# at-wat/mcl_3dl

Hardware: AMD Instinct MI355X
Metric: particle·point evals/sec; filter-update Hz @ 4096 particles × 16k-pt scan (higher is better)
Workload: dtype f32

## Files before the change

include/mcl3dl_hip.h:

```cpp
#ifndef MCL3DL_HIP_H
#define MCL3DL_HIP_H

#include <stddef.h>
#include <stdint.h>

#ifdef __cplusplus
extern "C" {
#endif

#define MCL3DL_HIP_ABI_VERSION 3

typedef struct mcl3dl_hip_ctx mcl3dl_hip_ctx;

enum
{
  MCL3DL_BEAM_SHORT = 0,
  MCL3DL_BEAM_HIT = 1,
  MCL3DL_BEAM_LONG = 2,
  MCL3DL_BEAM_TOTAL_REFLECTION = 3
};

enum
{
  MCL3DL_KERNEL_LIKELIHOOD = 0,
// ... 206 lines not shown
int mcl3dl_hip_group_measure_imu(mcl3dl_hip_group* g, const float* acc3, float acc_var, float* out_weight ,
                                 float* out_lik , float* entropy, int* restored);
int mcl3dl_hip_group_set_odom_error_sigma(mcl3dl_hip_group* g, float sigma);
int mcl3dl_hip_global_localization_rotations(int div_yaw, const float* imu_quat4 ,
                                             float* out_quat4 );
int mcl3dl_hip_global_localization_points(mcl3dl_hip_ctx* ctx, double grid, float* out_xyz ,
                                          size_t capacity, size_t* n_points, size_t* n_centroids);
int mcl3dl_hip_global_localization_seed_device(mcl3dl_hip_ctx* ctx, int div_yaw, const float* imu_quat4, size_t first,
                                               size_t count, float* d_state13, float* d_pose7, float* d_weight);
int mcl3dl_hip_group_global_localization(mcl3dl_hip_group* g, double grid, int div_yaw, const float* imu_quat4,
                                         size_t max_particles , size_t* n_points, size_t* n_particles);
int mcl3dl_hip_sampler_normal_direction(const float* mean7 , const float* cov36 ,
                                        double perform_weighting_ratio, double max_weight_ratio, double max_weight,
                                        float* out_fpc_local3, double* out_max_weight, double* out_eigen_value_ratio );
int mcl3dl_hip_scan_normal_weights(mcl3dl_hip_ctx* ctx, int which, double normal_search_range, const float* fpc_local3,
                                   double max_weight, double* out_cumulative , float* out_normal_xyz ,
                                   size_t capacity, size_t* n, size_t* n_without_normal );
int mcl3dl_hip_group_collective_stats(const mcl3dl_hip_group* g, uint64_t* rccl_all_reduces, uint64_t* host_combines);

int mcl3dl_hip_set_kernel_timing(mcl3dl_hip_ctx* ctx, int enable);
int mcl3dl_hip_get_kernel_time(mcl3dl_hip_ctx* ctx, int kernel_id, double* total_ms, uint64_t* launches);
int mcl3dl_hip_reset_kernel_time(mcl3dl_hip_ctx* ctx);
int mcl3dl_hip_workload_stats(mcl3dl_hip_ctx* ctx, const float* d_pose, size_t n_p, double* stats6);
int mcl3dl_hip_memory_footprint(mcl3dl_hip_ctx* ctx, uint64_t* bytes8);
int mcl3dl_hip_set_option(mcl3dl_hip_ctx* ctx, const char* name, double value);
int mcl3dl_hip_get_option(mcl3dl_hip_ctx* ctx, const char* name, double* value);
int mcl3dl_hip_index_stats(mcl3dl_hip_ctx* ctx, double* stats8);

#ifdef __cplusplus
}
#endif
#endif
```

mcl_3dl_amd/capi.py:

```python
import ctypes as C
import os

import numpy as np

_HERE = os.path.dirname(os.path.abspath(__file__))
LIB_PATH = os.environ.get("MCL3DL_HIP_LIB") or os.path.join(_HERE, "libmcl3dl_hip.so")

KERNEL_LIKELIHOOD, KERNEL_BEAM, KERNEL_PF, KERNEL_UPDATE, KERNEL_STAGE = 0, 1, 2, 3, 4
BEAM_STATUS = {0: "SHORT", 1: "HIT", 2: "LONG", 3: "TOTAL_REFLECTION"}

_f, _d, _sz, _u32, _u64, _i, _p = C.c_float, C.c_double, C.c_size_t, C.c_uint32, C.c_uint64, C.c_int, C.c_void_p

SIGNATURES = {
    "mcl3dl_hip_abi_version": (_i, []),
    "mcl3dl_hip_create": (_i, [C.POINTER(_p), _i]),
    "mcl3dl_hip_destroy": (None, [_p]),
    "mcl3dl_hip_last_error": (C.c_char_p, [_p]),
    "mcl3dl_hip_set_stream": (_i, [_p, _p]),
    "mcl3dl_hip_get_stream": (_p, [_p]),
    "mcl3dl_hip_synchronize": (_i, [_p]),
    "mcl3dl_hip_set_map": (_i, [_p, _p, _p, _sz, _u64, _p]),
    "mcl3dl_hip_set_likelihood_params": (_i, [_p, _f, _f, _f]),
    "mcl3dl_hip_set_beam_params": (_i, [_p, _f, _f, _f, _f, _f, _f, _f, _u32, _f, _u32, _i]),
    "mcl3dl_hip_set_beam_raycast": (_i, [_p, _i]),
# ... 17 lines not shown
    "mcl3dl_hip_expectation": (_i, [_p, _p, _p, _p, _sz, _p, _p, _p, _p]),
    "mcl3dl_hip_covariance": (_i, [_p, _p, _p, _sz, _p, _sz, _p, _p]),
    "mcl3dl_hip_expectation_device": (_i, [_p, _p, _p, _p, _sz, _p, _p, _p, _p]),
    "mcl3dl_hip_covariance_device": (_i, [_p, _p, _p, _sz, _p, _sz, _p, _p]),
    "mcl3dl_hip_resample_begin": (_i, [_p, _p, _sz, _sz, C.POINTER(_f)]),
    "mcl3dl_hip_resample_plan": (_i, [_p, _i, _f, _p, _p, C.POINTER(_sz)]),
    "mcl3dl_hip_resample_apply": (_i, [_p, _p, _p, _sz, _p]),
    "mcl3dl_hip_resample_apply_device": (_i, [_p, _p, _p, _sz, _p]),
    "mcl3dl_hip_moments_partial_device": (_i, [_p, _p, _p, _p, _sz, _p]),
    "mcl3dl_hip_moments_finish": (_i, [_p, _i, _p, _p, C.POINTER(_f), C.POINTER(C.c_int64), C.POINTER(C.c_int64)]),
    "mcl3dl_hip_covariance_partial_device": (_i, [_p, _p, _p, _sz, _p, _sz, _p, _p]),
    "mcl3dl_hip_covariance_finish": (_i, [_p, _p]),
    "mcl3dl_hip_update_device": (_i, [_p, _p, _sz, _p, _p, _p, _p, _p, _p]),
    "mcl3dl_hip_resample_begin_device": (_i, [_p, _p, _sz, _sz, C.POINTER(_f)]),
    "mcl3dl_hip_resample_apply_slice_device": (_i, [_p, _p, _p, _sz, _sz, _sz, _p]),
    "mcl3dl_hip_upload_scan": (_i, [_p, _p, _sz, _p, _p, _sz, _p, _sz]),
    "mcl3dl_hip_measure_device": (_i, [_p, _p, _sz, _p, _p, _p]),
    "mcl3dl_hip_pf_partial_device": (_i, [_p, _p, _p, _p, _p, _p, _sz, _i, _i, _p]),
    "mcl3dl_hip_pf_apply_device": (_i, [_p, _p, _sz, _i, _p, _p]),
    "mcl3dl_hip_set_kernel_timing": (_i, [_p, _i]),
    "mcl3dl_hip_get_kernel_time": (_i, [_p, _i, C.POINTER(_d), C.POINTER(_u64)]),
    "mcl3dl_hip_reset_kernel_time": (_i, [_p]),
    "mcl3dl_hip_workload_stats": (_i, [_p, _p, _sz, _p]),
    "mcl3dl_hip_memory_footprint": (_i, [_p, _p]),
    "mcl3dl_hip_set_option": (_i, [_p, C.c_char_p, _d]),
    "mcl3dl_hip_scan_begin": (_i, [_p, _p, _p, _sz, _p, _p, _p, C.POINTER(_sz), C.POINTER(_sz), C.POINTER(_sz)]),
    "mcl3dl_hip_scan_begin_pointcloud2": (_i, [_p, _p, _sz, _u32, _i, _i, _i, _i, _u32, _p, _p, _p, C.POINTER(_sz),
                                              C.POINTER(_sz), C.POINTER(_sz)]),
    "mcl3dl_hip_scan_finish": (_i, [_p, _p, _sz, _p, _sz, _p, _sz]),
    "mcl3dl_hip_scan_download": (_i, [_p, _i, _p, _p, _sz, C.POINTER(_sz)]),
    "mcl3dl_hip_set_map_pointcloud2": (_i, [_p, _p, _sz, _u32, _i, _i, _i, _i, _p, _u64, _p, C.POINTER(_sz)]),
    "mcl3dl_hip_set_map_downsampled": (_i, [_p, _p, _p, _sz, _p, _u64, _p, C.POINTER(_sz)]),
    "mcl3dl_hip_map_update": (_i, [_p, _p, _p, _sz, _p, _u64, C.POINTER(_sz), _p]),
    "mcl3dl_hip_map_update_pointcloud2": (_i, [_p, _p, _sz, _u32, _i, _i, _i, _i, _p, _u64, C.POINTER(_sz), _p]),
    "mcl3dl_hip_map_download": (_i, [_p, _p, _p, _sz, C.POINTER(_sz)]),
    "mcl3dl_hip_match_split": (_i, [_p, _p, _p, _sz, _f, _d, _p, _sz, C.POINTER(_sz), _p, _sz, C.POINTER(_sz)]),
    "mcl3dl_hip_group_create": (_i, [C.POINTER(_p), C.POINTER(_i), _i]),
    "mcl3dl_hip_group_destroy": (None, [_p]),
    "mcl3dl_hip_group_last_error": (C.c_char_p, [_p]),
    "mcl3dl_hip_group_size": (_i, [_p]),
    "mcl3dl_hip_group_context": (_p, [_p, _i]),
    "mcl3dl_hip_group_shard": (_i, [_sz, _i, _i, C.POINTER(_sz), C.POINTER(_sz)]),
    "mcl3dl_hip_group_set_map": (_i, [_p, _p, _p, _sz, _u64, _p]),
    "mcl3dl_hip_group_set_likelihood_params": (_i, [_p, _f, _f, _f]),
    "mcl3dl_hip_group_set_beam_params": (_i, [_p, _f, _f, _f, _f, _f, _f, _f, _u32, _f, _u32, _i]),
    "mcl3dl_hip_group_set_beam_raycast": (_i, [_p, _i]),
# ... 838 lines not shown
                                                          _ptr(d_extra), _ptr(d_ratio), n_p, int(rank), int(world),
                                                          _ptr(d_packed)))

    def pf_apply_device(self, d_weight, n_p, d_packed, d_stats4, world=1):
        self._check(self.lib.mcl3dl_hip_pf_apply_device(self.h, _ptr(d_weight), n_p, int(world), _ptr(d_packed),
                                                        _ptr(d_stats4)))

    def set_kernel_timing(self, enable):
        self._check(self.lib.mcl3dl_hip_set_kernel_timing(self.h, int(bool(enable))))

    def reset_kernel_time(self):
        self._check(self.lib.mcl3dl_hip_reset_kernel_time(self.h))

    def kernel_time(self, kernel_id):
        ms, n = C.c_double(0), C.c_uint64(0)
        self._check(self.lib.mcl3dl_hip_get_kernel_time(self.h, kernel_id, C.byref(ms), C.byref(n)))
        return float(ms.value), int(n.value)

    def workload_stats(self, d_pose, n_p):
        st = np.zeros(6, np.float64)
        self._check(self.lib.mcl3dl_hip_workload_stats(self.h, _ptr(d_pose), n_p, _ptr(st)))
        return dict(sum_k=st[0], evals=st[1], dda_steps=st[2], dda_occupied=st[3], dda_tested=st[4], rays=st[5])

    def memory_footprint(self):
        b = np.zeros(8, np.uint64)
        self._check(self.lib.mcl3dl_hip_memory_footprint(self.h, _ptr(b)))
        return dict(lik_points=int(b[0]), lik_cells=int(b[1]), dda_bits=int(b[2]), dda_voxels=int(b[3]),
                    dda_points=int(b[4]), cand_table=int(b[5]), cand_start=int(b[6]), cand_points=int(b[7]))

    def set_option(self, name, value):
        self._check(self.lib.mcl3dl_hip_set_option(self.h, name.encode(), float(value)))

    def get_option(self, name):
        v = C.c_double(0)
        self._check(self.lib.mcl3dl_hip_get_option(self.h, name.encode(), C.byref(v)))
        return float(v.value)

    def index_stats(self):
        s = np.zeros(8, np.float64)
        self._check(self.lib.mcl3dl_hip_index_stats(self.h, _ptr(s)))
        return dict(bricks=int(s[0]), preliminary=int(s[1]), candidates=int(s[2]), build_ms=float(s[3]),
                    voxels_with_candidates=int(s[4]), voxels_with_overflow=int(s[5]), overflow_records=int(s[6]),
                    voxel_ratio=float(s[7]), voxels_over8=int(self.get_option("cand_voxels_over8")),
                    record_parts=int(self.get_option("cand_record_parts_in_use")),
                    packed_words=int(self.get_option("cand_packed_active")),
                    deferred_overflow=int(self.get_option("lik_defer_active")))
# ... 1 lines not shown
```

mcl_3dl_amd/csrc/grid_kernels.h:

```cpp
#pragma once
#include <hip/hip_runtime.h>
#include <stdint.h>

#include "map_structs.h"
#pragma clang fp contract(off)

namespace mcl3dl
{
__global__ void grid_rescale_kernel(const float4* __restrict__ map, long long n, float wx, float wy, float wz, int has_weight,
                                    float4* __restrict__ out)
{
  const long long i = static_cast<long long>(blockIdx.x) * blockDim.x + threadIdx.x;
  if (i >= n)
    return;
  const float4 p = map[i];
  out[i] = make_float4(has_weight ? p.x * wx : p.x, has_weight ? p.y * wy : p.y, has_weight ? p.z * wz : p.z,
                       __uint_as_float(static_cast<uint32_t>(i)));
}

struct CellGeom
{
  float ox, oy, oz, inv;
  int nx, ny, nz;
};
// ... 181 lines not shown
  unsigned long long bit;
  dda_brick_bit(g, v, brick, bit);
  atomicAnd(&bricks[brick], ~bit);
}

__global__ void dda_overlay_set_kernel(const float4* __restrict__ upd, const uint32_t* __restrict__ skey,
                                       const uint32_t* __restrict__ sval, int n, DdaGeom g, uint32_t* __restrict__ ov_key,
                                       float4* __restrict__ ov_pts, uint32_t* __restrict__ ov_idx,
                                       unsigned long long* __restrict__ bricks)
{
  const int k = static_cast<int>(blockIdx.x * blockDim.x + threadIdx.x);
  if (k >= n)
    return;
  const uint32_t v = skey[k], i = sval[k];
  ov_key[k] = v;
  ov_pts[k] = upd[i];
  ov_idx[k] = i;
  size_t brick;
  unsigned long long bit;
  dda_brick_bit(g, v, brick, bit);
  atomicOr(&bricks[brick], bit);
}

}
```

mcl_3dl_amd/csrc/host_context.h:

```cpp
#pragma once

namespace
{
struct DevBuf
{
  void* p = nullptr;
  size_t cap = 0;
  bool view = false;
  DevBuf() = default;
  DevBuf(const DevBuf&) = delete;
  DevBuf& operator=(const DevBuf&) = delete;
  ~DevBuf()
  {
    if (p && !view)
      (void)hipFree(p);
  }
  template <typename T>
  T* as() const
  {
    return static_cast<T*>(p);
  }
};

struct OrderedScan
// ... 126 lines not shown
    for (const PinnedBlock& b : pinned)
      if (c >= b.p && c + bytes <= b.p + b.bytes)
        return true;
    return false;
  }
  double cand_voxel_ratio = 0.0;
  double cand_phase = 0.5;
  int cand_aniso = 2;
  bool cand_aniso_active = false;
  double cand_aniso_max = 8.0;
  double index_budget_opt = -1.0;
  double index_budget_bytes = 0.0;
  double cand_need_bytes = 0.0;
  double cand_edge_ratio[3] = { 0.5, 0.5, 0.5 };
  int cand_record_parts = 0;
  uint32_t cand_parts = 4;
  int n_cus = 256;
  int cand_packed = 1;
  int cand_bound = 1;
  int lik_defer = 1;
  double lik_defer_min_frac = 0.03;
  double cand_over8 = 0;
  DevBuf cand_table, cand_start, cand_pts, cand_rec, cand_ovf;
  DevBuf cand_all_pts;
  CompileParams cand_cp{};
  long long cand_n_table = 0;
  uint32_t cand_n_bricks = 0, cand_n_ovf = 0, cand_ovf_leaked = 0;
  uint64_t cand_ovf_compactions = 0;
  size_t cand_n_points = 0;
  RecGrid rg{};
  double cand_stats[8] = { 0, 0, 0, 0, 0, 0, 0, 0 };
  DevBuf dda_bits, dda_start, dda_pts, dda_index;
  DevBuf dda_ov_key, dda_ov_pts, dda_ov_idx;
  int dda_overlay = 1;
  bool dda_overlay_ok = false;
  uint64_t dda_overlay_updates = 0;
  DdaGeom dda_geom{};
  DevBuf map_dev;
  bool map_dev_valid = false;
  size_t map_dev_n = 0;
  int grid_build_host = 0;
  double grid_build_ms[2] = { 0, 0 };
  double grid_build_wall_ms[2] = { 0, 0 };
  DdaGrid dg{};
  uint64_t footprint[8] = { 0, 0, 0, 0, 0, 0, 0, 0 };

// ... 568 lines not shown
```

mcl_3dl_amd/csrc/host_map_compilers.h:

```cpp
#pragma once

namespace
{
int build_lik_grid(mcl3dl_hip_ctx* ctx);
int build_dda_grid(mcl3dl_hip_ctx* ctx);
int ensure_map_dev(mcl3dl_hip_ctx* ctx);
int cloud_minmax(mcl3dl_hip_ctx* ctx, const float4* pts, long long n, float* host6, unsigned long long* host_cnt);

void kd_ray_radii(const mcl3dl_hip_ctx* ctx, float* grid_min, float* r1, float* r2)
{
  const float mn = std::min({ ctx->map_grid[0], ctx->map_grid[1], ctx->map_grid[2] });
  const float mx = std::max({ ctx->map_grid[0], ctx->map_grid[1], ctx->map_grid[2] });
  *grid_min = mn;
  *r1 = static_cast<float>(std::sqrt(2.0) * mx / 2.0);
  *r2 = static_cast<float>(mn * 2 + std::sqrt(2.0) * mx / 2.0);
}

bool lik_cell_is_beams(const mcl3dl_hip_ctx* ctx)
{
  return !ctx->lik_params_set && ctx->beam_raycast == 1;
}

float lik_cell_edge(const mcl3dl_hip_ctx* ctx)
{
// ... 363 lines not shown
{
  sp.resize(count);
  for (size_t k = 0; k < count; ++k)
  {
    const size_t i = first + k;
    float v[3];
    for (int a = 0; a < 3; ++a)
    {
      v[a] = ctx->has_weight ? ctx->map_xyz[3 * i + a] * ctx->weight[a] : ctx->map_xyz[3 * i + a];
      if (!std::isfinite(v[a]))
        return ctx->fail(-3, "map point %zu is not finite", i);
      if (mn && (k == 0 || v[a] < mn[a]))
        mn[a] = v[a];
      if (mx && (k == 0 || v[a] > mx[a]))
        mx[a] = v[a];
    }
    sp[k] = make_float4(v[0], v[1], v[2], bits_to_float(static_cast<uint32_t>(i)));
  }
  return 0;
}

uint32_t bytes32(unsigned long long bytes)
{
  return bytes < (1ull << 32) ? static_cast<uint32_t>(bytes) : 0u;
}

void set_word_format(RecGrid& g, int fmt, float r)
{
  g.packed = fmt != 0 ? 1 : 0;
  g.count_shift = fmt == 2 ? REC2_COUNT_SHIFT : REC_EXT_BITS;
  g.ext_bits = fmt == 2 ? REC2_EXT_BITS : REC_EXT_BITS;
  g.count_is_records = fmt == 2 ? 1 : 0;
  g.over_thr = fmt == 2 ? (1u << REC2_COUNT_SHIFT) - 1u : ((4u << REC_EXT_BITS) | REC_EXT_MASK);
  g.bound_step = fmt == 2 ? r / static_cast<float>(REC2_BOUND_MAX) : 0.0f;
}

int word_format(const RecGrid& g)
{
  return !g.packed ? 0 : (g.bound_step > 0.0f ? 2 : 1);
}

struct CompileOutput
{
  unsigned long long total = 0, kept = 0;
  unsigned long long hist3[5] = { 0, 0, 0, 0, 0 };
  uint32_t n_ovf = 0;
  int packed = 0;
// ... 96 lines not shown
  if (want_packed >= 0)
    out->packed = want_packed;
  else
    out->packed = (can_bound && ctx->cand_packed && ctx->cand_bound) ? 2 : (can_pack && ctx->cand_packed) ? 1 : 0;
  TRY(scratch_alloc(ctx, out->d_ovf_data, 64ull * (n_ovf ? n_ovf : 1)));
  {
    const long long words = 16ll * (n_ovf ? n_ovf : 1);
    uint32_t sentinel_bits;
    const float sentinel = REC_SENTINEL;
    memcpy(&sentinel_bits, &sentinel, sizeof(sentinel_bits));
    hipLaunchKernelGGL(mc_fill_u32, dim3(static_cast<unsigned>((words + 255) / 256)), dim3(256), 0, ctx->stream,
                       static_cast<uint32_t*>(out->d_ovf_data.p), sentinel_bits, words);
  }
  hipLaunchKernelGGL(mc_write_records, dim3(blocks_v), dim3(256), 0, ctx->stream, pts,
                     static_cast<const uint32_t*>(d_pstart.p), static_cast<const uint32_t*>(d_prelim.p),
                     static_cast<const uint32_t*>(d_count.p), static_cast<const uint32_t*>(d_ovf.p), rec_out,
                     static_cast<float*>(out->d_ovf_data.p), n_vox, cap, out->packed, cp, bxyz,
                     static_cast<double>(ctx->match_dist_min));
  HIP_TRY(hipGetLastError());
  out->n_ovf = n_ovf;
  return 0;
}

constexpr int RC_OVER_BUDGET = 1;

int build_cand_grid_at(mcl3dl_hip_ctx* ctx, double voxel_ratio, uint32_t cap = 4)
{
  const unsigned long long rec_bytes = 16ull * cap;
  const size_t n = ctx->map_xyz.size() / 3;
  EventPairRaii evs;
  HIP_TRY(hipEventCreate(&evs.a));
  HIP_TRY(hipEventCreate(&evs.b));
  const hipEvent_t ev0 = evs.a, ev1 = evs.b;
  HIP_TRY(hipEventRecord(ev0, ctx->stream));
  TRY(ensure_map_dev(ctx));
  TRY(ensure(ctx, ctx->cand_all_pts, sizeof(float4) * n));
  hipLaunchKernelGGL(grid_rescale_kernel, dim3(static_cast<unsigned>((n + 255) / 256)), dim3(256), 0, ctx->stream,
                     ctx->map_dev.as<float4>(), static_cast<long long>(n), ctx->weight[0], ctx->weight[1], ctx->weight[2],
                     ctx->has_weight ? 1 : 0, ctx->cand_all_pts.as<float4>());
  float mm[6];
  unsigned long long n_finite = 0;
  TRY(cloud_minmax(ctx, ctx->cand_all_pts.as<float4>(), static_cast<long long>(n), mm, &n_finite));
  if (n_finite != n)
    return ctx->fail(-3, "%llu map point(s) are not finite", static_cast<unsigned long long>(n) - n_finite);
  const float* mn = mm;
  const float* mx = mm + 3;
// ... 7 lines not shown
  TempBuf d_flag, d_scan, d_bxyz;
  TRY(scratch_alloc(ctx, d_flag, sizeof(int) * n_table));
  TRY(scratch_alloc(ctx, d_scan, sizeof(uint32_t) * (n_table + 1)));
  HIP_TRY(hipMemsetAsync(d_flag.p, 0, sizeof(int) * n_table, ctx->stream));
  const float4* pts = ctx->cand_all_pts.as<float4>();
  hipLaunchKernelGGL(mc_mark_bricks, dim3(static_cast<unsigned>((n + 255) / 256)), dim3(256), 0, ctx->stream, cp, pts,
                     static_cast<int*>(d_flag.p));
  HIP_TRY(hipMemsetAsync(d_scan.p, 0, sizeof(uint32_t) * (n_table + 1), ctx->stream));
  HIP_TRY(hipMemcpyAsync(d_scan.p, d_flag.p, sizeof(int) * n_table, hipMemcpyDeviceToDevice, ctx->stream));
  TRY(device_exclusive_scan(ctx, static_cast<uint32_t*>(d_scan.p), n_table + 1));
  uint32_t n_bricks = 0;
  TRY(d2h(ctx, &n_bricks, static_cast<uint32_t*>(d_scan.p) + n_table, sizeof(uint32_t)));
  TRY(sync_stream(ctx));
  if (n_bricks == 0 || n_bricks > (1u << 22))
    return ctx->fail(-4, "candidate index: %u bricks", n_bricks);
  ctx->cand_need_bytes = static_cast<double>(rec_bytes) * 512.0 * n_bricks;
  if (ctx->lik_index == 2 && ctx->index_budget_bytes > 0.0 && ctx->cand_need_bytes > ctx->index_budget_bytes)
    return RC_OVER_BUDGET;
  TRY(ensure(ctx, ctx->cand_table, sizeof(int) * (n_table + 1)));
  int* table = ctx->cand_table.as<int>();
  hipLaunchKernelGGL(mc_brick_ids, dim3(static_cast<unsigned>((n_table + 255) / 256)), dim3(256), 0, ctx->stream,
                     static_cast<const int*>(d_flag.p), static_cast<const uint32_t*>(d_scan.p), table, n_table);
  HIP_TRY(hipMemsetAsync(table + n_table, 0xff, sizeof(int), ctx->stream));
  TRY(scratch_alloc(ctx, d_bxyz, sizeof(int) * 3 * n_bricks));
  hipLaunchKernelGGL(mc_brick_coords, dim3(static_cast<unsigned>((n_table + 255) / 256)), dim3(256), 0, ctx->stream,
                     table, cp.nbx, cp.nby, n_table, static_cast<int*>(d_bxyz.p));
  const long long n_vox = static_cast<long long>(n_bricks) * 512;
  const bool records = ctx->lik_index == 2;
  if (records)
    TRY(ensure(ctx, ctx->cand_rec, rec_bytes * static_cast<size_t>(n_vox)));
  CompileOutput co;
  TRY(compile_bricks(ctx, cp, pts, table, static_cast<const int*>(d_bxyz.p), n_bricks, records,
                     records ? ctx->cand_rec.as<float>() : nullptr, &co, cap));
  const unsigned long long total = co.total, kept = co.kept;
  ctx->cand_cp = cp;
  ctx->cand_n_table = n_table;
  ctx->cand_n_bricks = n_bricks;
  ctx->cand_n_points = n;
  if (records)
  {
    const uint32_t n_ovf = co.n_ovf;
    TRY(ensure(ctx, ctx->cand_ovf, 64ull * (n_ovf ? n_ovf : 1)));
    HIP_TRY(hipMemcpyAsync(ctx->cand_ovf.p, co.d_ovf_data.p, 64ull * (n_ovf ? n_ovf : 1), hipMemcpyDeviceToDevice,
                           ctx->stream));
    ctx->cand_n_ovf = n_ovf;
    ctx->cand_ovf_leaked = 0;
    HIP_TRY(hipEventRecord(ev1, ctx->stream));
    TRY(sync_stream(ctx));
    float ms2 = 0.f;
    HIP_TRY(hipEventSynchronize(ev1));
    HIP_TRY(hipEventElapsedTime(&ms2, ev0, ev1));
    RecGrid& g = ctx->rg;
    g.brick_table = table;
    g.rec = ctx->cand_rec.as<float4>();
    g.ovf = ctx->cand_ovf.as<float4>();
    g.ox = cp.ox;
    g.oy = cp.oy;
    g.oz = cp.oz;
    g.inv_ex = cp.inv_ex;
    g.inv_ey = cp.inv_ey;
    g.inv_ez = cp.inv_ez;
    g.nvx = cp.nvx;
    g.nvy = cp.nvy;
    g.nvz = cp.nvz;
    g.nbx = cp.nbx;
    g.nby = cp.nby;
    g.nbz = cp.nbz;
    g.mul24_ok = (static_cast<long long>(cp.nbx) * cp.nby < (1ll << 24) && cp.nbz < (1 << 24)) ? 1 : 0;
    g.off32_ok = (rec_bytes * static_cast<unsigned long long>(n_vox) < (1ull << 32)) ? 1 : 0;
    g.rec_bytes32 = bytes32(rec_bytes * static_cast<unsigned long long>(n_vox));
    g.rec_parts = static_cast<int>(cap);
    set_word_format(g, co.packed, ctx->match_dist_min);
    ctx->cand_parts = cap;
    g.ovf_bytes32 = bytes32(64ull * (n_ovf ? n_ovf : 1));
    g.ti_empty = static_cast<uint32_t>(n_table);
    ctx->footprint[5] = sizeof(int) * n_table;
    ctx->footprint[6] = rec_bytes * static_cast<size_t>(n_vox);
    ctx->footprint[7] = 64ull * n_ovf;
    ctx->cand_stats[0] = n_bricks;
    ctx->cand_stats[1] = static_cast<double>(total);
    ctx->cand_stats[2] = static_cast<double>(kept);
    ctx->cand_stats[3] = ms2;
    ctx->cand_stats[4] = static_cast<double>(co.hist3[0]);
    ctx->cand_stats[5] = static_cast<double>(co.hist3[1]);
    ctx->cand_over8 = static_cast<double>(co.hist3[2]);
    ctx->cand_stats[6] = n_ovf;
    ctx->cand_stats[7] = cp.ex / static_cast<double>(ctx->match_dist_min);
    ctx->cand_edge_ratio[0] = cp.ex / static_cast<double>(ctx->match_dist_min);
    ctx->cand_edge_ratio[1] = cp.ey / static_cast<double>(ctx->match_dist_min);
    ctx->cand_edge_ratio[2] = cp.ez / static_cast<double>(ctx->match_dist_min);
    ctx->cand_dirty = false;
    return 0;
  }
  return ctx->fail(-3, "the candidate index is built for lik_index = 2 only");
}

int build_cand_grid_budgeted(mcl3dl_hip_ctx* ctx, double ratio, uint32_t cap, double* ratio_used = nullptr)
{
  if (ctx->index_budget_opt < 0.0)
// ... 264 lines not shown
      if (stats5)
        stats5[5] = 7;
      ctx->cand_dirty = true;
      return 0;
    }
    if (rc != 0)
      return rc;
  }
  const uint32_t ovf_base = ctx->cand_n_ovf;
  if (co.n_ovf)
  {
    TRY(ensure_keep(ctx, ctx->cand_ovf, 64ull * ovf_base, 64ull * (static_cast<size_t>(ovf_base) + co.n_ovf)));
    HIP_TRY(hipMemcpyAsync(ctx->cand_ovf.as<char>() + 64ull * ovf_base, co.d_ovf_data.p, 64ull * co.n_ovf,
                           hipMemcpyDeviceToDevice, ctx->stream));
  }
  TempBuf d_orphan;
  TRY(scratch_alloc(ctx, d_orphan, sizeof(unsigned long long)));
  HIP_TRY(hipMemsetAsync(d_orphan.p, 0, sizeof(unsigned long long), ctx->stream));
  hipLaunchKernelGGL(mc_install_records, dim3(static_cast<unsigned>((n_sub_vox + 255) / 256)), dim3(256), 0, ctx->stream,
                     static_cast<const float4*>(d_subrec.p), static_cast<const int*>(d_sub_main.p), ovf_base, n_bricks_old,
                     n_sub_vox, ctx->cand_rec.as<float4>(), static_cast<unsigned long long*>(d_orphan.p), cap, ctx->rg.packed,
                     ctx->rg.count_shift, ctx->rg.count_is_records);
  HIP_TRY(hipGetLastError());
  unsigned long long orphaned = 0;
  TRY(d2h(ctx, &orphaned, d_orphan.p, sizeof(orphaned)));
  HIP_TRY(hipEventRecord(ev1, ctx->stream));
  TRY(sync_stream(ctx));
  float ms = 0.f;
  HIP_TRY(hipEventSynchronize(ev1));
  HIP_TRY(hipEventElapsedTime(&ms, ev0, ev1));
  ctx->cand_n_bricks = n_bricks;
  ctx->cand_n_ovf = ovf_base + co.n_ovf;
  ctx->cand_ovf_leaked += static_cast<uint32_t>(orphaned);
  ctx->cand_n_points = n_total;
  ctx->rg.brick_table = ctx->cand_table.as<int>();
  ctx->rg.rec = ctx->cand_rec.as<float4>();
  ctx->rg.ovf = ctx->cand_ovf.as<float4>();
  ctx->rg.off32_ok = (rec_bytes * 512 * n_bricks < (1ull << 32)) ? 1 : 0;
  ctx->rg.rec_bytes32 = bytes32(rec_bytes * 512 * n_bricks);
  ctx->rg.ovf_bytes32 = bytes32(64ull * (ctx->cand_n_ovf ? ctx->cand_n_ovf : 1));
  ctx->footprint[6] = rec_bytes * 512 * n_bricks;
  ctx->footprint[7] = 64ull * ctx->cand_n_ovf;
  ctx->cand_stats[0] = n_bricks;
  ctx->cand_stats[6] = ctx->cand_n_ovf;
  ++ctx->generation;
  if (stats5)
  {
    stats5[0] = n_dirty;
    stats5[1] = n_new;
    stats5[2] = n_rel;
    stats5[3] = ms;
    stats5[4] = co.n_ovf;
  }
  return 0;
}

}
```

mcl_3dl_amd/csrc/likelihood_kernels.h:

```cpp
#pragma once
#include <hip/hip_runtime.h>
#include <stdint.h>

#include "device_math.h"
#include "float_chain.h"
#include "map_structs.h"
#pragma clang fp contract(off)

namespace mcl3dl
{
template <bool STATS>
__device__ inline float nearest_d2(const LikGrid& g, float qx, float qy, float qz, unsigned& n_tested)
{
  const float fx = floorf((qx - g.ox) * g.inv_cell);
  const float fy = floorf((qy - g.oy) * g.inv_cell);
  const float fz = floorf((qz - g.oz) * g.inv_cell);
  float best = 3.0e38f;
  if (!(fx >= 1.0f && fy >= 1.0f && fz >= 1.0f && fx <= static_cast<float>(g.nx - 2) &&
        fy <= static_cast<float>(g.ny - 2) && fz <= static_cast<float>(g.nz - 2)))
    return best;
  const int cx = static_cast<int>(fx), cy = static_cast<int>(fy), cz = static_cast<int>(fz);
  uint32_t rs[9], re[9];
#pragma unroll
  for (int r = 0; r < 9; ++r)
// ... 84 lines not shown
__device__ inline int floor_to_int(float x)
{
  int r;
  asm("v_cvt_flr_i32_f32 %0, %1" : "=v"(r) : "v"(x));
  return r;
}

__device__ inline bool rec_locate(const RecGrid& g, float qx, float qy, float qz, uint32_t& ti, uint32_t& sub)
{
  const int vx = floor_to_int((qx - g.ox) * g.inv_ex);
  const int vy = floor_to_int((qy - g.oy) * g.inv_ey);
  const int vz = floor_to_int((qz - g.oz) * g.inv_ez);
  if (g.mul24_ok)
    ti = __umul24(static_cast<uint32_t>(vz >> 3), static_cast<uint32_t>(g.nbx * g.nby)) +
         __umul24(static_cast<uint32_t>(vy >> 3), static_cast<uint32_t>(g.nbx)) + static_cast<uint32_t>(vx >> 3);
  else
    ti = (static_cast<uint32_t>(vz >> 3) * static_cast<uint32_t>(g.nby) + static_cast<uint32_t>(vy >> 3)) *
             static_cast<uint32_t>(g.nbx) + static_cast<uint32_t>(vx >> 3);
  sub = ((((static_cast<uint32_t>(vz) & 7u) << 3) | (static_cast<uint32_t>(vy) & 7u)) << 3) | (static_cast<uint32_t>(vx) & 7u);
  return static_cast<unsigned>(vx) < static_cast<unsigned>(g.nvx) && static_cast<unsigned>(vy) < static_cast<unsigned>(g.nvy) &&
         static_cast<unsigned>(vz) < static_cast<unsigned>(g.nvz);
}

__device__ inline float rec_overflow_min(const RecGrid& g, float qx, float qy, float qz, uint32_t n_records, uint32_t ext,
                                         float best)
{
  const float4* o = g.ovf + 4 * static_cast<size_t>(ext);
  for (uint32_t j = 0; j < 4u * n_records; ++j)
  {
    const float4 c = o[j];
    const float d = d2_simple(qx, qy, qz, c.x, c.y, c.z);
    best = d < best ? d : best;
  }
  return best;
}

template <bool STATS>
__device__ inline float nearest_d2_rec(const RecGrid& g, float qx, float qy, float qz, unsigned& n_tested)
{
  float best = 3.0e38f;
  uint32_t ti, sub;
  if (!rec_locate(g, qx, qy, qz, ti, sub))
    return best;
  const int b = g.brick_table[ti];
  if (b < 0)
    return best;
// ... 217 lines not shown
      best = (more && m < best) ? m : best;
    }
  }
  return best;
}

__device__ inline float sqrt_in_radius(float x)
{
  float s = __builtin_amdgcn_sqrtf(x);
  const float s_dn = __uint_as_float(__float_as_uint(s) - 1u), s_up = __uint_as_float(__float_as_uint(s) + 1u);
  const float vp = __builtin_fmaf(-s_dn, s, x), vs = __builtin_fmaf(-s_up, s, x);
  s = (vp <= 0.0f) ? s_dn : s;
  s = (vs > 0.0f) ? s_up : s;
  return s;
}

__device__ inline float eval_coop(const RecGrid& rg, const LikParams& prm, const Vec3f pos, const Quat rot, const float4 v,
                                  bool have_point, int lane, bool& matched)
{
  const Vec3f tp = vadd(qrot_trim(rot, Vec3f{ v.x, v.y, v.z }), pos);
  const float qx = tp.x * prm.wx, qy = tp.y * prm.wy, qz = tp.z * prm.wz;
  uint32_t ti, sub;
  const bool inside = rec_locate(rg, qx, qy, qz, ti, sub) && have_point;
  const int b = rg.brick_table[inside ? ti : rg.ti_empty];
  const bool valid = b >= 0;
  float dist = -1.0f;
  if (wave_any(valid))
  {
    const uint32_t rec = (static_cast<uint32_t>(b) << 9) | sub;
    const uint32_t vrec = rg.rec_bytes32 ? rec : (valid ? rec : 0u);
    const float d2 = rec_min_d2_quad(rg, qx, qy, qz, vrec, valid, lane);
    if (valid && d2 < prm.r2)
    {
      const float s = sqrt_in_radius(d2);
      dist = lik_dist(prm, s);
    }
  }
  matched = !(dist < 0.0f);
  return lik_term(prm, dist, matched);
}

template <int BLOCK, int MODE, bool STATS>
__device__ __forceinline__ void lik_particle(const Vec3f pos, const Quat rot, const float4* __restrict__ scan, int n_s,
                                             const LikGrid& g, const RecGrid& rg, const LikParams& prm,
                                             int coop, double& sum_out, unsigned& num_out, unsigned& tested_out,
                                             const uint32_t* __restrict__ perm = nullptr, float* s_row = nullptr)
{
  double acc = 0.0;
  unsigned num = 0;
  unsigned tested = 0;
  const bool rows = !STATS && s_row != nullptr;
  if (rows)
  {
    if (static_cast<int>(threadIdx.x) < chain_row_floats(n_s) - n_s)
      s_row[n_s + threadIdx.x] = 0.0f;
// ... 222 lines not shown

__device__ inline unsigned long long chain_pack(uint32_t value, uint32_t tag)
{
  return (static_cast<unsigned long long>(tag) << 32) | value;
}

constexpr int CHAIN_POLL_MAX = 1 << 20;
constexpr int DEFER_QCAP = 96;

struct DeferQueue
{
  uint32_t word[4][DEFER_QCAP];
  uint16_t who[4][DEFER_QCAP];
};

__device__ inline float eval_coop_first(const RecGrid& rg, const LikParams& prm, const Vec3f pos, const Quat rot, const float4 v,
                                        bool have_point, int lane, bool& matched, bool& over, float& best, uint32_t& mine,
                                        unsigned long long& over_m)
{
  const Vec3f tp = vadd(qrot_trim(rot, Vec3f{ v.x, v.y, v.z }), pos);
  const float qx = tp.x * prm.wx, qy = tp.y * prm.wy, qz = tp.z * prm.wz;
  uint32_t ti, sub;
  const bool inside = rec_locate(rg, qx, qy, qz, ti, sub) && have_point;
  const int b = rg.brick_table[inside ? ti : rg.ti_empty];
  const bool valid = b >= 0;
  float dist = -1.0f;
  over = false;
  over_m = 0ull;
  best = 0.0f;
  mine = 0u;
  const unsigned long long valid_m = __builtin_amdgcn_ballot_w64(valid);
  if (valid_m != 0ull)
  {
    const uint32_t rec = (static_cast<uint32_t>(b) << 9) | sub;
    const uint32_t vrec = rg.rec_bytes32 ? rec : (valid ? rec : 0u);
    uint32_t w[4];
    best = quad_round(rg.rec, rg.rec_bytes32, vrec, qx, qy, qz, lane & 3, w);
    mine = own_word(w, lane & 3);
    over_m = valid_m & lanes_gt_u32(mine, rg.over_thr);
    if (rg.bound_step > 0.0f && over_m != 0ull)
    {
      asm volatile("");
      over_m &= __builtin_amdgcn_fcmpf(best, rec_bound2(rg, mine), 2 );
    }
    over = __builtin_amdgcn_inverse_ballot_w64(over_m);
    if (valid && !over && best < prm.r2)
    {
      const float s = sqrt_in_radius(best);
      dist = lik_dist(prm, s);
    }
  }
  matched = !(dist < 0.0f);
  return lik_term(prm, dist, matched);
}

template <int G, int LD>
__device__ inline void defer_drain(const RecGrid& rg, const LikParams& prm, const float (&s_pose)[G][8], float (&s_term)[G][LD],
                                   unsigned (&s_cnt)[G][4], const DeferQueue& q, int wave, int lane, uint32_t base, uint32_t n,
                                   const float4 v)
{
  const bool act = static_cast<uint32_t>(lane) < n;
  const uint32_t slot = act ? base + static_cast<uint32_t>(lane) : base;
  const uint32_t word = q.word[wave][slot];
  const uint32_t who = q.who[wave][slot];
  const int src = static_cast<int>(who & 63u), k = static_cast<int>(who >> 6);
  const Vec3f pt = { __shfl(v.x, src), __shfl(v.y, src), __shfl(v.z, src) };
  const Vec3f pos = { s_pose[k][0], s_pose[k][1], s_pose[k][2] };
  const Quat rot = { s_pose[k][3], s_pose[k][4], s_pose[k][5], s_pose[k][6] };
  const Vec3f tp = vadd(qrot_trim(rot, pt), pos);
// ... 495 lines not shown
```

mcl_3dl_amd/csrc/map_compiler.h:

```cpp
#pragma once
#include <hip/hip_runtime.h>
#include <stdint.h>

namespace mcl3dl
{
struct CompileParams
{
  float ox, oy, oz, inv_ex, inv_ey, inv_ez;
  double ex, ey, ez;
  double grow;
  double r2_hi;
  double margin;
  int rx, ry, rz;
  int nvx, nvy, nvz, nbx, nby, nbz;
  int n_points;
};

__device__ inline int3 voxel_of(const CompileParams& c, const float4 p)
{
  return make_int3(static_cast<int>(floorf((p.x - c.ox) * c.inv_ex)), static_cast<int>(floorf((p.y - c.oy) * c.inv_ey)),
                   static_cast<int>(floorf((p.z - c.oz) * c.inv_ez)));
}

__device__ inline long long brick_index(const CompileParams& c, int vx, int vy, int vz)
// ... 485 lines not shown
        kept_count[v] = n;
    }
    __syncthreads();
  }
}


constexpr float REC_SENTINEL = 1.0e18f;
constexpr uint32_t REC_EXT_BITS = 26u, REC_EXT_MASK = (1u << REC_EXT_BITS) - 1u, REC_COUNT_MAX = 63u;
constexpr uint32_t REC2_EXT_BITS = 22u, REC2_COUNT_SHIFT = 28u, REC2_BOUND_MAX = 63u;

struct RecGrid
{
  const int32_t* brick_table;
  const float4* rec;
  const float4* ovf;
  float ox, oy, oz, inv_ex, inv_ey, inv_ez;
  int nvx, nvy, nvz, nbx, nby, nbz;
  int mul24_ok;
  int off32_ok;
  uint32_t rec_bytes32, ovf_bytes32;
  int rec_parts;
  uint32_t ti_empty;
  int packed;
  uint32_t count_shift, ext_bits;
  int count_is_records;
  uint32_t over_thr;
  float bound_step;
};

__host__ __device__ inline uint32_t rec_ext_mask(const RecGrid& g)
{
  return (1u << g.ext_bits) - 1u;
}
__host__ __device__ inline uint32_t rec_overflow_records(uint32_t field, uint32_t cap, int count_is_records)
{
  return count_is_records ? field : (field > cap ? (field - cap + 3u) / 4u : 0u);
}
__device__ inline float rec_bound2(const RecGrid& g, uint32_t w)
{
  const float bd = static_cast<float>((w >> REC2_EXT_BITS) & REC2_BOUND_MAX) * g.bound_step;
  return bd * bd;
}

__global__ __launch_bounds__(256) void mc_count_overflow(const uint32_t* __restrict__ kept_count, uint32_t* __restrict__ n_ovf,
                                                         long long n_vox, unsigned long long* __restrict__ hist3, uint32_t cap)
// ... 81 lines not shown
    {
      if (k == 0)
        o.w = __uint_as_float(c);
      if (k == 1)
        o.w = __uint_as_float(c > cap ? ovf_start[v] : 0u);
    }
    dst[k] = o;
  }
  if (c > cap)
  {
    float* o = ovf + 16 * static_cast<size_t>(ovf_start[v]);
    for (uint32_t k = cap; k < c; ++k)
    {
      const float4 p = pts[prelim[src + k] & 0x7fffffffu];
      const uint32_t j = k - cap;
      float* slot = o + 4 * j;
      slot[0] = p.x;
      slot[1] = p.y;
      slot[2] = p.z;
    }
  }
}

__global__ void mc_new_brick_flags(const int* __restrict__ dirty, const int* __restrict__ table, uint32_t* __restrict__ new_flag,
                                   long long n_table)
{
  const long long i = static_cast<long long>(blockIdx.x) * blockDim.x + threadIdx.x;
  if (i > n_table)
    return;
  new_flag[i] = (i < n_table && dirty[i] && table[i] < 0) ? 1u : 0u;
}

__global__ void mc_dirty_tables(const int* __restrict__ dirty, const uint32_t* __restrict__ new_rank,
                                const uint32_t* __restrict__ dirty_rank, uint32_t n_bricks_old, int nbx, int nby,
                                long long n_table, int* __restrict__ table, int* __restrict__ sub_table,
                                int* __restrict__ sub_main, int* __restrict__ sub_bxyz)
{
  const long long i = static_cast<long long>(blockIdx.x) * blockDim.x + threadIdx.x;
  if (i >= n_table)
    return;
  if (!dirty[i])
  {
    sub_table[i] = -1;
    return;
  }
  int id = table[i];
// ... 203 lines not shown
```

Measured before the change: 301.9 billion.

## Add per-brick 64-bit occupancy masks to skip empty 2x2x2 voxel blocks

Builds a 64-bit mask per brick marking which 2x2x2 voxel blocks contain any kept points. The likelihood kernels then read this mask and leave lanes whose block is empty out of the live set, so the record gather and distance rounds are skipped when a wave has no live lanes. The cost is an extra 8-byte-per-table-entry buffer, an extra global load per query, and a mask build kernel at compile and update time. It also adds a stats kernel and API for counting empty-brick, empty-block and empty-voxel queries, and tightens the bytes32 limit.

```diff
diff --git a/include/mcl3dl_hip.h b/include/mcl3dl_hip.h
--- a/include/mcl3dl_hip.h
+++ b/include/mcl3dl_hip.h
@@ -252,6 +252,7 @@
 int mcl3dl_hip_get_kernel_time(mcl3dl_hip_ctx* ctx, int kernel_id, double* total_ms, uint64_t* launches);
 int mcl3dl_hip_reset_kernel_time(mcl3dl_hip_ctx* ctx);
 int mcl3dl_hip_workload_stats(mcl3dl_hip_ctx* ctx, const float* d_pose, size_t n_p, double* stats6);
+int mcl3dl_hip_index_query_stats(mcl3dl_hip_ctx* ctx, const float* d_pose, size_t n_p, double* stats4);
 int mcl3dl_hip_memory_footprint(mcl3dl_hip_ctx* ctx, uint64_t* bytes8);
 int mcl3dl_hip_set_option(mcl3dl_hip_ctx* ctx, const char* name, double value);
 int mcl3dl_hip_get_option(mcl3dl_hip_ctx* ctx, const char* name, double* value);
diff --git a/mcl_3dl_amd/capi.py b/mcl_3dl_amd/capi.py
--- a/mcl_3dl_amd/capi.py
+++ b/mcl_3dl_amd/capi.py
@@ -63,6 +63,7 @@
     "mcl3dl_hip_get_kernel_time": (_i, [_p, _i, C.POINTER(_d), C.POINTER(_u64)]),
     "mcl3dl_hip_reset_kernel_time": (_i, [_p]),
     "mcl3dl_hip_workload_stats": (_i, [_p, _p, _sz, _p]),
+    "mcl3dl_hip_index_query_stats": (_i, [_p, _p, _sz, _p]),
     "mcl3dl_hip_memory_footprint": (_i, [_p, _p]),
     "mcl3dl_hip_set_option": (_i, [_p, C.c_char_p, _d]),
     "mcl3dl_hip_scan_begin": (_i, [_p, _p, _p, _sz, _p, _p, _p, C.POINTER(_sz), C.POINTER(_sz), C.POINTER(_sz)]),
@@ -947,6 +948,11 @@
         self._check(self.lib.mcl3dl_hip_workload_stats(self.h, _ptr(d_pose), n_p, _ptr(st)))
         return dict(sum_k=st[0], evals=st[1], dda_steps=st[2], dda_occupied=st[3], dda_tested=st[4], rays=st[5])
 
+    def index_query_stats(self, d_pose, n_p):
+        st = np.zeros(4, np.float64)
+        self._check(self.lib.mcl3dl_hip_index_query_stats(self.h, _ptr(d_pose), n_p, _ptr(st)))
+        return dict(evals=st[0], no_brick=st[1], empty_block=st[2], empty_voxel=st[3])
+
     def memory_footprint(self):
         b = np.zeros(8, np.uint64)
         self._check(self.lib.mcl3dl_hip_memory_footprint(self.h, _ptr(b)))
diff --git a/mcl_3dl_amd/csrc/grid_kernels.h b/mcl_3dl_amd/csrc/grid_kernels.h
--- a/mcl_3dl_amd/csrc/grid_kernels.h
+++ b/mcl_3dl_amd/csrc/grid_kernels.h
@@ -227,4 +227,42 @@
   atomicOr(&bricks[brick], bit);
 }
 
-}
+__global__ __launch_bounds__(256) void index_query_stats_kernel(const float* __restrict__ pose7, const float4* __restrict__ scan,
+                                                                int n_s, RecGrid rg, const unsigned long long* __restrict__ mask,
+                                                                LikParams prm, unsigned long long* __restrict__ out4)
+{
+  const float* ps = pose7 + 7 * static_cast<size_t>(blockIdx.x);
+  const Vec3f pos = { ps[0], ps[1], ps[2] };
+  const Quat rot = qnormalized(Quat{ ps[3], ps[4], ps[5], ps[6] });
+  unsigned n_out = 0, n_block = 0, n_voxel = 0;
+  for (int i = threadIdx.x; i < n_s; i += 256)
+  {
+    const float4 v = scan[i];
+    const Vec3f tp = vadd(qrot_trim(rot, Vec3f{ v.x, v.y, v.z }), pos);
+    uint32_t ti, sub;
+    const bool inside = rec_locate(rg, tp.x * prm.wx, tp.y * prm.wy, tp.z * prm.wz, ti, sub);
+    const int b = inside ? rg.brick_table[ti] : -1;
+    if (b < 0)
+    {
+      ++n_out;
+      continue;
+    }
+    const uint32_t block = (((sub >> 7) & 3u) << 4) | (((sub >> 4) & 3u) << 2) | ((sub >> 1) & 3u);
+    n_block += ((mask[ti] >> block) & 1ull) ? 0u : 1u;
+    const size_t rec = static_cast<size_t>(rg.rec_parts) * ((static_cast<uint32_t>(b) << 9) | sub);
+    n_voxel += rg.rec[rec].x == REC_SENTINEL ? 1u : 0u;
+  }
+  n_out = wave_sum(n_out);
+  n_block = wave_sum(n_block);
+  n_voxel = wave_sum(n_voxel);
+  if ((threadIdx.x & 63) == 0)
+  {
+    if (threadIdx.x == 0)
+      atomicAdd(&out4[0], static_cast<unsigned long long>(n_s));
+    atomicAdd(&out4[1], static_cast<unsigned long long>(n_out));
+    atomicAdd(&out4[2], static_cast<unsigned long long>(n_block));
+    atomicAdd(&out4[3], static_cast<unsigned long long>(n_voxel));
+  }
+}
+
+}
diff --git a/mcl_3dl_amd/csrc/host_context.h b/mcl_3dl_amd/csrc/host_context.h
--- a/mcl_3dl_amd/csrc/host_context.h
+++ b/mcl_3dl_amd/csrc/host_context.h
@@ -172,6 +172,8 @@
   double lik_defer_min_frac = 0.03;
   double cand_over8 = 0;
   DevBuf cand_table, cand_start, cand_pts, cand_rec, cand_ovf;
+  DevBuf cand_mask;
+  int brick_mask = 1;
   DevBuf cand_all_pts;
   CompileParams cand_cp{};
   long long cand_n_table = 0;
diff --git a/mcl_3dl_amd/csrc/host_map_compilers.h b/mcl_3dl_amd/csrc/host_map_compilers.h
--- a/mcl_3dl_amd/csrc/host_map_compilers.h
+++ b/mcl_3dl_amd/csrc/host_map_compilers.h
@@ -409,7 +409,7 @@
 
 uint32_t bytes32(unsigned long long bytes)
 {
-  return bytes < (1ull << 32) ? static_cast<uint32_t>(bytes) : 0u;
+  return bytes <= (1ull << 32) - 65536ull ? static_cast<uint32_t>(bytes) : 0u;
 }
 
 void set_word_format(RecGrid& g, int fmt, float r)
@@ -552,6 +552,18 @@
   return 0;
 }
 
+int write_brick_masks(mcl3dl_hip_ctx* ctx, const CompileParams& cp, const CompileOutput& co, const int* bxyz, uint32_t n_bricks,
+                      long long n_table)
+{
+  if (n_bricks == 0)
+    return 0;
+  hipLaunchKernelGGL(mc_brick_masks, dim3((n_bricks + 3u) / 4u), dim3(256), 0, ctx->stream,
+                     static_cast<const uint32_t*>(co.d_count.p), bxyz, n_bricks, cp.nbx, cp.nby, n_table,
+                     ctx->cand_mask.as<unsigned long long>());
+  HIP_TRY(hipGetLastError());
+  return 0;
+}
+
 constexpr int RC_OVER_BUDGET = 1;
 
 int build_cand_grid_at(mcl3dl_hip_ctx* ctx, double voxel_ratio, uint32_t cap = 4)
@@ -605,6 +617,9 @@
   hipLaunchKernelGGL(mc_brick_ids, dim3(static_cast<unsigned>((n_table + 255) / 256)), dim3(256), 0, ctx->stream,
                      static_cast<const int*>(d_flag.p), static_cast<const uint32_t*>(d_scan.p), table, n_table);
   HIP_TRY(hipMemsetAsync(table + n_table, 0xff, sizeof(int), ctx->stream));
+  TRY(ensure(ctx, ctx->cand_mask, sizeof(uint64_t) * (n_table + 1)));
+  HIP_TRY(hipMemsetAsync(ctx->cand_mask.p, 0, sizeof(uint64_t) * (n_table + 1), ctx->stream));
+  ctx->rg.brick_mask = nullptr;
   TRY(scratch_alloc(ctx, d_bxyz, sizeof(int) * 3 * n_bricks));
   hipLaunchKernelGGL(mc_brick_coords, dim3(static_cast<unsigned>((n_table + 255) / 256)), dim3(256), 0, ctx->stream,
                      table, cp.nbx, cp.nby, n_table, static_cast<int*>(d_bxyz.p));
@@ -615,6 +630,8 @@
   CompileOutput co;
   TRY(compile_bricks(ctx, cp, pts, table, static_cast<const int*>(d_bxyz.p), n_bricks, records,
                      records ? ctx->cand_rec.as<float>() : nullptr, &co, cap));
+  if (records)
+    TRY(write_brick_masks(ctx, cp, co, static_cast<const int*>(d_bxyz.p), n_bricks, n_table));
   const unsigned long long total = co.total, kept = co.kept;
   ctx->cand_cp = cp;
   ctx->cand_n_table = n_table;
@@ -657,7 +674,8 @@
     ctx->cand_parts = cap;
     g.ovf_bytes32 = bytes32(64ull * (n_ovf ? n_ovf : 1));
     g.ti_empty = static_cast<uint32_t>(n_table);
-    ctx->footprint[5] = sizeof(int) * n_table;
+    g.brick_mask = ctx->brick_mask ? ctx->cand_mask.as<uint64_t>() : nullptr;
+    ctx->footprint[5] = (sizeof(int) + sizeof(uint64_t)) * n_table;
     ctx->footprint[6] = rec_bytes * static_cast<size_t>(n_vox);
     ctx->footprint[7] = 64ull * n_ovf;
     ctx->cand_stats[0] = n_bricks;
@@ -968,6 +986,7 @@
                      n_sub_vox, ctx->cand_rec.as<float4>(), static_cast<unsigned long long*>(d_orphan.p), cap, ctx->rg.packed,
                      ctx->rg.count_shift, ctx->rg.count_is_records);
   HIP_TRY(hipGetLastError());
+  TRY(write_brick_masks(ctx, cp, co, static_cast<const int*>(d_sub_bxyz.p), n_dirty, n_table));
   unsigned long long orphaned = 0;
   TRY(d2h(ctx, &orphaned, d_orphan.p, sizeof(orphaned)));
   HIP_TRY(hipEventRecord(ev1, ctx->stream));
@@ -980,6 +999,7 @@
   ctx->cand_ovf_leaked += static_cast<uint32_t>(orphaned);
   ctx->cand_n_points = n_total;
   ctx->rg.brick_table = ctx->cand_table.as<int>();
+  ctx->rg.brick_mask = ctx->brick_mask ? ctx->cand_mask.as<uint64_t>() : nullptr;
   ctx->rg.rec = ctx->cand_rec.as<float4>();
   ctx->rg.ovf = ctx->cand_ovf.as<float4>();
   ctx->rg.off32_ok = (rec_bytes * 512 * n_bricks < (1ull << 32)) ? 1 : 0;
diff --git a/mcl_3dl_amd/csrc/likelihood_kernels.h b/mcl_3dl_amd/csrc/likelihood_kernels.h
--- a/mcl_3dl_amd/csrc/likelihood_kernels.h
+++ b/mcl_3dl_amd/csrc/likelihood_kernels.h
@@ -130,6 +130,19 @@
          static_cast<unsigned>(vz) < static_cast<unsigned>(g.nvz);
 }
 
+__device__ inline unsigned long long rec_block_lanes(const RecGrid& g, uint32_t ti, uint32_t sub)
+{
+  const uint64_t m = g.brick_mask[ti];
+  const uint32_t block = (((sub >> 7) & 3u) << 4) | (((sub >> 4) & 3u) << 2) | ((sub >> 1) & 3u);
+  return __builtin_amdgcn_uicmp(static_cast<uint32_t>(m >> block) & 1u, 0u, 33 );
+}
+
+__device__ inline uint32_t rec_index_or_dead(const RecGrid& g, int b, uint32_t sub, bool live)
+{
+  const uint32_t rec = (static_cast<uint32_t>(live ? b : -1) << 9) | sub;
+  return g.rec_bytes32 ? rec : (live ? rec : 0u);
+}
+
 __device__ inline float rec_overflow_min(const RecGrid& g, float qx, float qy, float qz, uint32_t n_records, uint32_t ext,
                                          float best)
 {
@@ -393,15 +406,22 @@
   const float qx = tp.x * prm.wx, qy = tp.y * prm.wy, qz = tp.z * prm.wz;
   uint32_t ti, sub;
   const bool inside = rec_locate(rg, qx, qy, qz, ti, sub) && have_point;
-  const int b = rg.brick_table[inside ? ti : rg.ti_empty];
-  const bool valid = b >= 0;
+  const uint32_t te = inside ? ti : rg.ti_empty;
+  const int b = rg.brick_table[te];
+  unsigned long long occ_m = ~0ull;
+  if (rg.brick_mask != nullptr)
+  {
+    asm volatile("");
+    occ_m = rec_block_lanes(rg, te, sub);
+  }
+  const unsigned long long live_m = __builtin_amdgcn_ballot_w64(b >= 0) & occ_m;
+  const bool live = __builtin_amdgcn_inverse_ballot_w64(live_m);
   float dist = -1.0f;
-  if (wave_any(valid))
-  {
-    const uint32_t rec = (static_cast<uint32_t>(b) << 9) | sub;
-    const uint32_t vrec = rg.rec_bytes32 ? rec : (valid ? rec : 0u);
-    const float d2 = rec_min_d2_quad(rg, qx, qy, qz, vrec, valid, lane);
-    if (valid && d2 < prm.r2)
+  if (live_m != 0ull)
+  {
+    const uint32_t vrec = rec_index_or_dead(rg, b, sub, live);
+    const float d2 = rec_min_d2_quad(rg, qx, qy, qz, vrec, live, lane);
+    if (live && d2 < prm.r2)
     {
       const float s = sqrt_in_radius(d2);
       dist = lik_dist(prm, s);
@@ -670,29 +690,35 @@
   const float qx = tp.x * prm.wx, qy = tp.y * prm.wy, qz = tp.z * prm.wz;
   uint32_t ti, sub;
   const bool inside = rec_locate(rg, qx, qy, qz, ti, sub) && have_point;
-  const int b = rg.brick_table[inside ? ti : rg.ti_empty];
-  const bool valid = b >= 0;
+  const uint32_t te = inside ? ti : rg.ti_empty;
+  const int b = rg.brick_table[te];
+  unsigned long long occ_m = ~0ull;
+  if (rg.brick_mask != nullptr)
+  {
+    asm volatile("");
+    occ_m = rec_block_lanes(rg, te, sub);
+  }
   float dist = -1.0f;
   over = false;
   over_m = 0ull;
   best = 0.0f;
   mine = 0u;
-  const unsigned long long valid_m = __builtin_amdgcn_ballot_w64(valid);
-  if (valid_m != 0ull)
-  {
-    const uint32_t rec = (static_cast<uint32_t>(b) << 9) | sub;
-    const uint32_t vrec = rg.rec_bytes32 ? rec : (valid ? rec : 0u);
+  const unsigned long long live_m = __builtin_amdgcn_ballot_w64(b >= 0) & occ_m;
+  const bool live = __builtin_amdgcn_inverse_ballot_w64(live_m);
+  if (live_m != 0ull)
+  {
+    const uint32_t vrec = rec_index_or_dead(rg, b, sub, live);
     uint32_t w[4];
     best = quad_round(rg.rec, rg.rec_bytes32, vrec, qx, qy, qz, lane & 3, w);
     mine = own_word(w, lane & 3);
-    over_m = valid_m & lanes_gt_u32(mine, rg.over_thr);
+    over_m = live_m & lanes_gt_u32(mine, rg.over_thr);
     if (rg.bound_step > 0.0f && over_m != 0ull)
     {
       asm volatile("");
       over_m &= __builtin_amdgcn_fcmpf(best, rec_bound2(rg, mine), 2 );
     }
     over = __builtin_amdgcn_inverse_ballot_w64(over_m);
-    if (valid && !over && best < prm.r2)
+    if (live && !over && best < prm.r2)
     {
       const float s = sqrt_in_radius(best);
       dist = lik_dist(prm, s);
diff --git a/mcl_3dl_amd/csrc/map_compiler.h b/mcl_3dl_amd/csrc/map_compiler.h
--- a/mcl_3dl_amd/csrc/map_compiler.h
+++ b/mcl_3dl_amd/csrc/map_compiler.h
@@ -531,6 +531,7 @@
   uint32_t rec_bytes32, ovf_bytes32;
   int rec_parts;
   uint32_t ti_empty;
+  const uint64_t* brick_mask;
   int packed;
   uint32_t count_shift, ext_bits;
   int count_is_records;
@@ -658,6 +659,26 @@
   }
 }
 
+__global__ __launch_bounds__(256) void mc_brick_masks(const uint32_t* __restrict__ kept_count, const int* __restrict__ brick_xyz,
+                                                      uint32_t n_bricks, int nbx, int nby, long long n_table,
+                                                      unsigned long long* __restrict__ mask)
+{
+  const uint32_t b = blockIdx.x * 4u + (threadIdx.x >> 6);
+  const uint32_t lane = threadIdx.x & 63u;
+  if (b >= n_bricks)
+    return;
+  const uint32_t x0 = (lane & 3u) << 1, y0 = ((lane >> 2) & 3u) << 1, z0 = (lane >> 4) << 1;
+  const uint32_t* c = kept_count + (static_cast<size_t>(b) << 9);
+  uint32_t any = 0;
+#pragma unroll
+  for (uint32_t k = 0; k < 8; ++k)
+    any |= c[((z0 + (k >> 2)) << 6) | ((y0 + ((k >> 1) & 1u)) << 3) | (x0 + (k & 1u))];
+  const unsigned long long m = __ballot(any != 0u);
+  const long long ti = (static_cast<long long>(brick_xyz[3 * b + 2]) * nby + brick_xyz[3 * b + 1]) * nbx + brick_xyz[3 * b + 0];
+  if (lane == 0 && ti >= 0 && ti < n_table)
+    mask[ti] = m;
+}
+
 __global__ void mc_new_brick_flags(const int* __restrict__ dirty, const int* __restrict__ table, uint32_t* __restrict__ new_flag,
                                    long long n_table)
 {
```

Result: slower. 290.3 billion (-3.9%).
